# Dongwon-Lee/gkmQC

Measured on AMD Instinct MI355X. Metric: gkm kernel pairs/sec (N=10k, 300 bp, L=11,k=7,d=3), higher is better.
Workload: dtype u32

## Files before the change

gkmqc_amd/csrc/bitslice_cpu_probe.cpp:

```cpp
#include <stdint.h>
#include <stdlib.h>
#include <algorithm>
#include <vector>

#include "gkm_bitslice.h"
#include "gkm_pack.h"

using namespace gkmbs;

template <int W, int L, int D>
static void run_pair(const uint8_t *A, int lenA, const uint8_t *B, int lenB, const uint8_t *wd,
                     uint32_t *acc )
{
    constexpr int NB = planes_for(D);
    constexpr int CAP = segment_capacity(W, L);
    const int nA = lenA - L + 1, nB = lenB - L + 1, T = lenB;
    for (int k = 0; k <= D; k++) acc[k] = 0;
    (void)NB;
    std::vector<uint32_t> sb[2][3];
    for (int st = 0; st < 2; st++)
        for (int pl = 0; pl < 3; pl++) {
            sb[st][pl].resize((size_t)T + W);
            for (int x = 0; x < T + W; x++) sb[st][pl][(size_t)x] = sb_word(B, T, st, x, W, L, pl);
        }
// ... 15 lines not shown
        uint32_t lanepk[2 * W + 2];
        for (int x = 0; x < 2 * W + 2; x++) {
            uint32_t v = 0u;
            for (int k = 0; k < 16; k++) {
                const int pos = s0 + x * 16 + k;
                if (x * 16 + k < 32 * W && pos < lenA) v |= (uint32_t)A[pos] << (2 * k);
            }
            lanepk[x] = v;
        }
        auto rl = [&](int i0) { return pk_window(lanepk[i0 >> 4], lanepk[(i0 >> 4) + 1], i0); };
        auto cl = [&](int st, int q) { return pk_window(pkB[st][(size_t)(q >> 4)], pkB[st][(size_t)(q >> 4) + 1], q); };
        const int c0 = nA / 2 - s0;
        for (int st = 0; st < 2; st++)
            for (int delta = 0; delta < T; delta++) {
                uint32_t hit[W];
                window_hits<W, L, D>(Ahi, Alo, AV, &sb[st][0][(size_t)delta], &sb[st][1][(size_t)delta],
                                     (delta & 1) ? (const uint32_t *)nullptr : &sb[st][2][(size_t)delta], hit);
                for (int w = 0; w < W; w++) {
                    uint32_t h = hit[w];
                    while (h) {
                        const int bit = __builtin_ctz(h);
                        h &= h - 1u;
                        const HitValue hv = resolve_hit_packed<W>(bit, w, delta, st, (uint32_t)T, rcpT, nB, L, c0, rl, cl, wdist);
                        if (hv.m <= D) acc[hv.m] += hv.v;
                    }
                }
            }
    }
}

#define CASE(WW, LL, DD) \
    if (W == WW && L == LL && d == DD) { run_pair<WW, LL, DD>(A, lenA, B, lenB, wd, acc); ok = 1; }

extern "C" int bsprobe_profile(int W, int L, int d, const uint8_t *A, int lenA, const uint8_t *B, int lenB,
                               const uint8_t *wd, int32_t *P)
{
    uint32_t acc[16] = {0};
    int ok = 0;
    CASE(10, 11, 3) CASE(10, 10, 3) CASE(10, 12, 4) CASE(10, 8, 4) CASE(10, 9, 4) CASE(10, 12, 6) CASE(10, 11, 5) CASE(10, 12, 5)
    CASE(10, 4, 2) CASE(10, 2, 1) CASE(10, 3, 0) CASE(10, 5, 2) CASE(10, 6, 3) CASE(10, 7, 3)
    CASE(5, 11, 3) CASE(16, 11, 3) CASE(3, 12, 4) CASE(10, 12, 8) CASE(10, 12, 12) CASE(10, 11, 1)
    CASE(10, 9, 5) CASE(10, 10, 5) CASE(10, 10, 6) CASE(10, 11, 6) CASE(10, 11, 7) CASE(10, 12, 7)
    if (!ok) return 1;
    for (int m = 0; m <= d; m++) P[m] = (int32_t)acc[m];
    return 0;
}

template <int W, int L, int D, int GRP>
static void run_group_any(const uint32_t *Ahi, const uint32_t *Alo, const uint32_t *AV, const uint32_t *Bhi, const uint32_t *Blo,
                          uint32_t *hit_or, uint32_t *any)
{
    uint32_t hit[W];
    window_hits<W, L, D>(Ahi, Alo, AV, Bhi, Blo, (const uint32_t *)nullptr, hit);
    for (int g = 0; g < W / GRP; g++) {
        hit_or[g] = 0u;
        for (int k = 0; k < GRP; k++) hit_or[g] |= hit[g * GRP + k];
    }
    window_group_any<W, L, D, GRP>(Ahi, Alo, AV, Bhi, Blo, any);
}

#define GCASE(LL, DD) \
    if (L == LL && d == DD) { run_group_any<10, LL, DD, 5>(Ahi, Alo, AV, Bhi, Blo, hit_or, any); *top_plane = top_plane_serves(LL, DD) ? 1 : 0; return 0; }
#define GCASE_L(LL) GCASE(LL, 0) GCASE(LL, 1) GCASE(LL, 2) GCASE(LL, 3) GCASE(LL, 4)

extern "C" int bsprobe_group_any(int L, int d, const uint32_t *Ahi, const uint32_t *Alo, const uint32_t *AV, const uint32_t *Bhi,
                                 const uint32_t *Blo, uint32_t *hit_or, uint32_t *any, int *top_plane)
{
    GCASE_L(5) GCASE_L(6) GCASE_L(7) GCASE_L(8) GCASE_L(9) GCASE_L(10) GCASE_L(11) GCASE_L(12)
    GCASE(11, 5) GCASE(12, 5) GCASE(12, 6)
    return 1;
}

template <int W, int L, int D, int GRP>
static int run_group_any_grouped(const uint32_t *Ahi, const uint32_t *Alo, const uint32_t *AV, const uint32_t *Bhi,
                                 const uint32_t *Blo, uint32_t *any_grouped, uint32_t *top_or, uint32_t *avg)
{
    if constexpr (!top_plane_serves(L, D)) {
        return 2;
    } else {
        uint32_t ones[W];
        for (int w = 0; w < W; w++) ones[w] = 0xFFFFFFFFu;
        window_group_any<W, L, D, GRP>(Ahi, Alo, ones, Bhi, Blo, top_or);
        for (int g = 0; g < W / GRP; g++) {
            avg[g] = 0u;
            for (int k = 0; k < GRP; k++) avg[g] |= AV[g * GRP + k];
        }
        window_group_any_grouped<W, L, D, GRP>(Ahi, Alo, avg, Bhi, Blo, any_grouped);
        return 0;
    }
}

#define GGCASE(LL, DD) \
    if (L == LL && d == DD) return run_group_any_grouped<10, LL, DD, 5>(Ahi, Alo, AV, Bhi, Blo, any_grouped, top_or, avg);
#define GGCASE_L(LL) GGCASE(LL, 0) GGCASE(LL, 1) GGCASE(LL, 2) GGCASE(LL, 3) GGCASE(LL, 4)

extern "C" int bsprobe_group_any_grouped(int L, int d, const uint32_t *Ahi, const uint32_t *Alo, const uint32_t *AV,
                                         const uint32_t *Bhi, const uint32_t *Blo, uint32_t *any_grouped, uint32_t *top_or,
                                         uint32_t *avg)
{
    GGCASE_L(5) GGCASE_L(6) GGCASE_L(7) GGCASE_L(8) GGCASE_L(9) GGCASE_L(10) GGCASE_L(11) GGCASE_L(12)
    GGCASE(11, 5) GGCASE(12, 5) GGCASE(12, 6)
    return 1;
}

template <int W, int L, int D, int GRP>
static int run_group_any_crossings(const uint32_t *Ahi, const uint32_t *Alo, const uint32_t *AVg, const uint32_t *Bhi,
                                   const uint32_t *Blo, uint32_t *any_grouped, uint32_t *any_crossings, uint32_t *any_one_way)
{
    if constexpr (!top_plane_serves(L, D)) {
        return 2;
    } else {
        window_group_any_grouped<W, L, D, GRP>(Ahi, Alo, AVg, Bhi, Blo, any_grouped);
        window_group_any_crossings<W, L, D, GRP>(Ahi, Alo, AVg, Bhi, Blo, any_crossings);
        window_group_any_crossings<W, L, D, GRP, false>(Ahi, Alo, AVg, Bhi, Blo, any_one_way);
        return 0;
    }
}

#define XCASE(LL, DD) \
    if (L == LL && d == DD) return run_group_any_crossings<10, LL, DD, 5>(Ahi, Alo, AVg, Bhi, Blo, any_grouped, any_crossings, any_one_way);
#define XCASE_L(LL) XCASE(LL, 0) XCASE(LL, 1) XCASE(LL, 2) XCASE(LL, 3) XCASE(LL, 4)

extern "C" int bsprobe_group_any_crossings(int L, int d, const uint32_t *Ahi, const uint32_t *Alo, const uint32_t *AVg,
                                           const uint32_t *Bhi, const uint32_t *Blo, uint32_t *any_grouped,
                                           uint32_t *any_crossings, uint32_t *any_one_way)
{
    XCASE_L(5) XCASE_L(6) XCASE_L(7) XCASE_L(8) XCASE_L(9) XCASE_L(10) XCASE_L(11) XCASE_L(12)
    XCASE(11, 5) XCASE(12, 5) XCASE(12, 6)
    return 1;
}

template <int W, int L, int D, int GRP>
static int run_group_any_centres(const uint32_t *Ahi, const uint32_t *Alo, const uint32_t *AVg, const uint32_t *Bhi,
                                 const uint32_t *Blo, uint32_t *any_grouped, uint32_t *any_centres)
{
    if constexpr (!top_plane_serves(L, D)) {
        return 2;
    } else {
        window_group_any_grouped<W, L, D, GRP>(Ahi, Alo, AVg, Bhi, Blo, any_grouped);
        window_group_any_centres<W, L, D, GRP>(Ahi, Alo, AVg, Bhi, Blo, any_centres);
        return 0;
    }
}

#define CCASE(LL, DD) \
    if (L == LL && d == DD) return run_group_any_centres<10, LL, DD, 5>(Ahi, Alo, AVg, Bhi, Blo, any_grouped, any_centres);
#define CCASE_L(LL) CCASE(LL, 0) CCASE(LL, 1) CCASE(LL, 2) CCASE(LL, 3) CCASE(LL, 4)

extern "C" int bsprobe_group_any_centres(int L, int d, const uint32_t *Ahi, const uint32_t *Alo, const uint32_t *AVg,
                                         const uint32_t *Bhi, const uint32_t *Blo, uint32_t *any_grouped, uint32_t *any_centres)
{
    CCASE_L(5) CCASE_L(6) CCASE_L(7) CCASE_L(8) CCASE_L(9) CCASE_L(10) CCASE_L(11) CCASE_L(12)
    CCASE(11, 5) CCASE(12, 5) CCASE(12, 6)
    return 1;
}

extern "C" void bsprobe_row_planes(const uint8_t *codes, int len, int s0, int W, int L, uint32_t *out)
{
    for (int pl = 0; pl < 3; pl++)
        for (int w = 0; w < W; w++) out[pl * W + w] = row_plane_word(codes, len, s0, w, W, L, pl);
}
extern "C" void bsprobe_sb_words(const uint8_t *codes, int T, int strand, int W, int L, int nx, uint32_t *hi, uint32_t *lo)
{
    for (int x = 0; x < nx; x++) {
        hi[x] = sb_word(codes, T, strand, x, W, L, 0);
        lo[x] = sb_word(codes, T, strand, x, W, L, 1);
    }
}
extern "C" void bsprobe_piece_valid(int b0, int nb, int cnt, int W, uint32_t *out)
{
    for (int w = 0; w < W; w++) {
        out[w] = 0u;
        for (int b = 0; b < 32; b++) out[w] |= piece_bit((const uint8_t *)nullptr, 0, b0, nb, 0, cnt, b, w, W, 2) << b;
    }
}

template <int W, int L, int D>
static int run_packed(const uint8_t *codes, const int64_t *off, const int *rows, int nrows, int col,
                      const uint8_t *wd, int32_t *P_out, int *lanes_used, int max_rows = gkmpack::MAX_ROWS, int own_mult = 1,
                      int rider_w = 0, int shift_trip = 0, long long *visits_out = nullptr)
{
    using namespace gkmpack;
    std::vector<int> nwin((size_t)nrows);
    for (int i = 0; i < nrows; i++) nwin[(size_t)i] = (int)(off[rows[i] + 1] - off[rows[i]]) - L + 1;
    const Packing P = pack_rows(rows, nwin.data(), nrows, W, L, max_rows, 0, own_mult, rider_w);
    *lanes_used = (int)P.lanes_used;
    std::vector<std::vector<int>> owned((size_t)nrows);
    for (int i = 0; i < nrows; i++) owned[(size_t)i].assign((size_t)nwin[(size_t)i], 0);
    std::vector<int> row_tile((size_t)nrows, -1);
    std::vector<int> lane_bits((size_t)P.ntiles * LANES, 0), lane_np((size_t)P.ntiles * LANES, 0);
    for (const Piece &pc : P.pieces) {
        if (pc.b0 < 0 || pc.nb <= 0 || pc.b0 + pc.nb > 32) return -1;
        if (pc.cnt <= 0 || pc.cnt > pc.nb * W - (L - 1)) return -2;
        if (pc.rider ? pc.b0 < lane_bits[(size_t)pc.lane] : pc.b0 != lane_bits[(size_t)pc.lane]) return -3;
        lane_bits[(size_t)pc.lane] = pc.b0 + pc.nb;
        if (++lane_np[(size_t)pc.lane] > MAX_PIECES) return -4;
        const int t = pc.lane / LANES;
        const int i = P.tile_out[(size_t)t * MAX_ROWS + pc.slot];
        if (i < 0 || i >= nrows || rows[i] != pc.row || P.tile_row[(size_t)t * MAX_ROWS + pc.slot] != pc.row) return -5;
        if (row_tile[(size_t)i] >= 0 && row_tile[(size_t)i] != t) return -6;
        row_tile[(size_t)i] = t;
        for (int k = 0; k < pc.cnt; k++) {
            if (pc.p0 + k >= nwin[(size_t)i]) return -7;
            owned[(size_t)i][(size_t)(pc.p0 + k)]++;
        }
    }
    for (int i = 0; i < nrows; i++)
        for (int v : owned[(size_t)i])
            if (v != 1) return -8;
    for (int t = 0; t < P.ntiles; t++)
        if (P.tile_nrows[(size_t)t] > MAX_ROWS) return -9;

    constexpr int NB = planes_for(D);
    (void)NB;
    const uint8_t *B = codes + off[col];
    const int T = (int)(off[col + 1] - off[col]), nB = T - L + 1;
    std::vector<uint32_t> sb[2][2];
    for (int st = 0; st < 2; st++)
        for (int pl = 0; pl < 2; pl++) {
            sb[st][pl].resize((size_t)T + W);
            for (int x = 0; x < T + W; x++) sb[st][pl][(size_t)x] = sb_word(B, T, st, x, W, L, pl);
        }
    auto wdist = [&](int Dd) { return wd ? (uint32_t)wd[Dd] : 1u; };
    const int pkw = (T + 15) / 16 + 1;
    std::vector<uint32_t> pkB[2];
    for (int st = 0; st < 2; st++) {
        pkB[st].resize((size_t)pkw);
        for (int x = 0; x < pkw; x++) pkB[st][(size_t)x] = pk_word(B, T, st, x);
    }
    const uint32_t rcpT = mod_magic((uint32_t)T);
    std::vector<uint32_t> acc((size_t)nrows * (D + 1), 0u);
    size_t pi = 0;
    while (pi < P.pieces.size()) {
        size_t pj = pi;
        while (pj < P.pieces.size() && P.pieces[pj].lane == P.pieces[pi].lane) pj++;
        uint32_t Ahi[W], Alo[W], AV[W], start_mask = 0u;
        uint32_t lanepk[2 * W + 2];
        for (int w = 0; w < W; w++) Ahi[w] = Alo[w] = AV[w] = 0u;
        for (int x = 0; x < 2 * W + 2; x++) lanepk[x] = 0u;
        for (size_t k = pi; k < pj; k++) {
            const Piece &pc = P.pieces[k];
            start_mask |= 1u << pc.b0;
            const uint8_t *seq = codes + off[pc.row];
            const int len = (int)(off[pc.row + 1] - off[pc.row]);
            for (int w = 0; w < W; w++)
                for (int b = 0; b < 32; b++) {
                    Ahi[w] |= piece_bit(seq, len, pc.b0, pc.nb, pc.p0, pc.cnt, b, w, W, 0) << b;
                    Alo[w] |= piece_bit(seq, len, pc.b0, pc.nb, pc.p0, pc.cnt, b, w, W, 1) << b;
                    AV[w] |= piece_bit(seq, len, pc.b0, pc.nb, pc.p0, pc.cnt, b, w, W, 2) << b;
                    const int i = b * W + w;
                    lanepk[i >> 4] |= ((piece_bit(seq, len, pc.b0, pc.nb, pc.p0, pc.cnt, b, w, W, 0) << 1) |
                                       piece_bit(seq, len, pc.b0, pc.nb, pc.p0, pc.cnt, b, w, W, 1)) << (2 * (i & 15));
                }
        }
        auto resolve = [&](int bit, int w, int delta, int st) -> int {
                        const Piece &pc = P.pieces[pi + (size_t)piece_of_bitrow(start_mask, bit)];
                        const uint8_t *seq = codes + off[pc.row];
                        const int len = (int)(off[pc.row + 1] - off[pc.row]), nA = len - L + 1;
                        auto rl = [&](int i0) { return pk_window(lanepk[i0 >> 4], lanepk[(i0 >> 4) + 1], i0); };
                        auto cl = [&](int s2, int q) { return pk_window(pkB[s2][(size_t)(q >> 4)], pkB[s2][(size_t)(q >> 4) + 1], q); };
                        const int c0 = nA / 2 - pc.p0 + pc.b0 * W;
                        (void)seq;
                        const HitValue hv = resolve_hit_packed<W>(bit, w, delta, st, (uint32_t)T, rcpT, nB, L, c0, rl, cl, wdist);
                        const int i = P.tile_out[(size_t)(pc.lane / LANES) * MAX_ROWS + pc.slot];
                        if (hv.m <= D) acc[(size_t)i * (D + 1) + hv.m] += hv.v;
                        else if (hv.v != 0u) return -20;
                        return 0;
        };
        if constexpr (W == 2 * SHIFT_GROUP_WORDS) {
            if (shift_trip > 0) {
                struct Rec { uint32_t any0, any1, origin; };
                uint32_t AVg[2] = {0u, 0u};
                for (int w = 0; w < W; w++) AVg[w / SHIFT_GROUP_WORDS] |= AV[w];
                for (int st = 0; st < 2; st++) {
                    std::vector<Rec> stack;
                    auto trip = [&](size_t c) -> int {
                        std::vector<Rec> top(stack.end() - (long)c, stack.end());
                        stack.resize(stack.size() - c);
                        for (Rec r : top) {
                            const ShiftVisit v = shift_record_visit(r.any0, r.any1);
                            const int delta = rec_delta(r.origin);
                            if (rec_w(r.origin) != 0) return -21;
                            uint32_t hit[W];
                            window_hits<W, L, D>(Ahi, Alo, AV, &sb[st][0][(size_t)delta], &sb[st][1][(size_t)delta],
                                                 (const uint32_t *)nullptr, hit);
                            for (int k = 0; k < SHIFT_GROUP_WORDS; k++)
                                if ((hit[v.w0 + k] >> v.bit) & 1u)
                                    if (const int rc = resolve((int)v.bit, (int)v.w0 + k, delta, st)) return rc;
                            if (visits_out) visits_out[1]++;
                            if (shift_record_live(r.any0, r.any1)) {
                                stack.push_back(r);
                                if (visits_out) visits_out[2]++;
                            }
                        }
                        return 0;
                    };
                    for (int delta = 0; delta < T; delta++) {
                        uint32_t any[2];
                        if constexpr (top_plane_serves(L, D))
                            window_group_any_centres<W, L, D, SHIFT_GROUP_WORDS>(Ahi, Alo, AVg, &sb[st][0][(size_t)delta],
                                                                                 &sb[st][1][(size_t)delta], any);
                        else
                            window_group_any<W, L, D, SHIFT_GROUP_WORDS>(Ahi, Alo, AV, &sb[st][0][(size_t)delta],
                                                                         &sb[st][1][(size_t)delta], any);
                        if (shift_record_live(any[0], any[1])) {
                            stack.push_back(Rec{any[0], any[1], pack_meta(delta, 0, 0)});
// ... 198 lines not shown
```

gkmqc_amd/csrc/gkm_bitslice.h:

```cpp
#ifndef GKM_BITSLICE_H
#define GKM_BITSLICE_H

#include <stdint.h>

#if defined(__HIPCC__)
#define GKM_HD __host__ __device__ __forceinline__
#else
#define GKM_HD inline
#endif

namespace gkmbs {

constexpr int planes_for(int d) { return d <= 1 ? 1 : d <= 3 ? 2 : d <= 7 ? 3 : 4; }

constexpr int segment_capacity(int W, int L) { return 32 * W - (L - 1); }

template <int TT>
GKM_HD uint32_t lop3(uint32_t a, uint32_t b, uint32_t c)
{
#if defined(__HIP_DEVICE_COMPILE__)
    return __builtin_amdgcn_bitop3_b32(a, b, c, TT);
#else
    uint32_t r = 0u;
    for (int k = 0; k < 8; k++)
// ... 285 lines not shown
                const uint32_t zout = Z[w - 1], zin = Z[w + L - 1];
                const uint32_t old0 = cnt.b[0];
                cnt.b[0] = lop3<TT_XOR3>(old0, zin, zout);
                uint32_t t = lop3<TT_BXC_AND_AXC>(old0, zin, zout);
#pragma unroll
                for (int i = 1; i < P; i++) {
                    const uint32_t old = cnt.b[i];
                    cnt.b[i] = old ^ t;
                    if (i + 1 < P) t = lop3<TT_A_AND_BXC>(t, old, zout);
                }
            }
            const uint32_t top = cnt.b[P - 1];
            if (w % GRP == 0) any[w / GRP] = top & AV[w];
            else any[w / GRP] = lop3<TT_A_OR_BC>(any[w / GRP], top, AV[w]);
        }
    }
}

template <int W, int L, int D, int GRP>
GKM_HD void window_group_any_grouped(const uint32_t *Ahi, const uint32_t *Alo, const uint32_t *AVg, const uint32_t *Bhi,
                                     const uint32_t *Blo, uint32_t *any)
{
    static_assert(L >= 2 && L <= 12, "L out of range");
    static_assert(W % GRP == 0, "a shift is a whole number of groups");
    static_assert(top_plane_serves(L, D), "the grouped form exists for the top-plane (L, D) pairs only");
    constexpr int P = bitlen(L);
    constexpr int BETA = top_plane_bias(L, D);
    constexpr int NX = W + L - 1;
    uint32_t Z[NX];
#pragma unroll
    for (int w = 0; w < W; w++) Z[w] = lop3<TT_NOT_A_OR_BXC>(Ahi[w] ^ Bhi[w], Alo[w], Blo[w]);
#pragma unroll
    for (int x = W; x < NX; x++) Z[x] = Z[x - W] >> 1;

    Cnt<P, L + BETA> cnt;
    static_assert(Cnt<P, L + BETA>::P == P && !Cnt<P, L + BETA>::OV, "the biased count fills exactly its planes");
    cnt.ovf = 0u;
    plane_sum_columns_biased<0, P, L + BETA, L, BETA == 1>(Z, cnt);
    uint32_t top[W];
#pragma unroll
    for (int w = 0; w < W; w++) {
        if (w > 0) {
            const uint32_t zout = Z[w - 1], zin = Z[w + L - 1];
            const uint32_t old0 = cnt.b[0];
            cnt.b[0] = lop3<TT_XOR3>(old0, zin, zout);
            uint32_t t = lop3<TT_BXC_AND_AXC>(old0, zin, zout);
#pragma unroll
            for (int i = 1; i < P; i++) {
                const uint32_t old = cnt.b[i];
                cnt.b[i] = old ^ t;
                if (i + 1 < P) t = lop3<TT_A_AND_BXC>(t, old, zout);
            }
        }
        top[w] = cnt.b[P - 1];
        if (w % GRP == GRP - 1) {
            const int w0 = w - (GRP - 1);
            uint32_t a = top[w0];
#pragma unroll
            for (int g = 1; g + 1 < GRP; g += 2) a = lop3<TT_OR3>(a, top[w0 + g], top[w0 + g + 1]);
            if (GRP % 2 == 0) a |= top[w0 + GRP - 1];
            any[w0 / GRP] = a & AVg[w0 / GRP];
        }
    }
}

constexpr int TT_AXB_OR_C = 0xBE;
constexpr int TT_AB_AND_C = 0xA8;

template <int P>
GKM_HD uint32_t count_step_crossing(uint32_t *lo, uint32_t zin, uint32_t zout, bool last)
{
    const uint32_t old0 = lo[0];
    if (!last) lo[0] = lop3<TT_XOR3>(old0, zin, zout);
    uint32_t t = lop3<TT_BXC_AND_AXC>(old0, zin, zout);
#pragma unroll
    for (int i = 1; i < P - 1; i++) {
        const uint32_t old = lo[i];
        if (!last) lo[i] = old ^ t;
        t = lop3<TT_A_AND_BXC>(t, old, zout);
    }
    return t;
}
template <int N>
GKM_HD uint32_t or_terms_and(uint32_t a, const uint32_t *t, uint32_t v)
{
#pragma unroll
    for (int i = 0; i + 1 < N; i += 2) a = lop3<TT_OR3>(a, t[i], t[i + 1]);
    if constexpr (N % 2 == 1) return lop3<TT_AB_AND_C>(a, t[N - 1], v);
    else return a & v;
}

template <int W, int L, int D, int GRP, bool MIDDLE = true>
GKM_HD void window_group_any_crossings(const uint32_t *Ahi, const uint32_t *Alo, const uint32_t *AVg, const uint32_t *Bhi,
                                       const uint32_t *Blo, uint32_t *any)
{
    static_assert(L >= 2 && L <= 12, "L out of range");
    static_assert(W == 2 * GRP && GRP >= 3, "a shift is two groups");
    static_assert(top_plane_serves(L, D), "the crossings form exists for the top-plane (L, D) pairs only");
    constexpr int P = bitlen(L);
    static_assert(P >= 2, "a top plane and at least one below it");
    constexpr int BETA = top_plane_bias(L, D);
    constexpr int NX = W + L - 1;
    constexpr int C = MIDDLE ? GRP : 0;
    uint32_t Z[NX];
#pragma unroll
    for (int w = 0; w < W; w++) Z[w] = lop3<TT_NOT_A_OR_BXC>(Ahi[w] ^ Bhi[w], Alo[w], Blo[w]);
#pragma unroll
    for (int x = W; x < NX; x++) Z[x] = Z[x - W] >> 1;

    Cnt<P, L + BETA> cnt;
    static_assert(Cnt<P, L + BETA>::P == P && !Cnt<P, L + BETA>::OV, "the biased count fills exactly its planes");
    cnt.ovf = 0u;
    plane_sum_columns_biased<0, P, L + BETA, L, BETA == 1>(Z + C, cnt);
    const uint32_t top = cnt.b[P - 1];
    uint32_t up[P - 1];
#pragma unroll
    for (int i = 0; i < P - 1; i++) up[i] = cnt.b[i];

    if constexpr (MIDDLE) {
        uint32_t dn[P - 1];
#pragma unroll
        for (int i = 0; i < P - 1; i++) dn[i] = cnt.b[i];
        uint32_t tu[GRP - 1], td[GRP];
#pragma unroll
        for (int s = 0; s < GRP - 1; s++) {
            const int w = C + 1 + s;
            tu[s] = count_step_crossing<P>(up, Z[w + L - 1], Z[w - 1], s == GRP - 2);
        }
#pragma unroll
        for (int s = 0; s < GRP; s++) {
            const int w = C - 1 - s;
            td[s] = count_step_crossing<P>(dn, Z[w], Z[w + L], s == GRP - 1);
        }
        any[1] = or_terms_and<GRP - 1>(top, tu, AVg[1]);
        any[0] = or_terms_and<GRP - 2>(lop3<TT_AXB_OR_C>(top, td[0], td[1]), td + 2, AVg[0]);
    } else {
        uint32_t t[W - 1];
#pragma unroll
        for (int w = 1; w < W; w++) t[w - 1] = count_step_crossing<P>(up, Z[w + L - 1], Z[w - 1], w == W - 1);
        any[0] = or_terms_and<GRP - 1>(top, t, AVg[0]);
        uint32_t e = top;
#pragma unroll
        for (int i = 0; i + 1 < GRP; i += 2) e = lop3<TT_XOR3>(e, t[i], t[i + 1]);
        if constexpr (GRP % 2 == 0) any[1] = or_terms_and<GRP - 1>(e, t + GRP, AVg[1]);
        else any[1] = or_terms_and<GRP - 2>(lop3<TT_AXB_OR_C>(e, t[GRP - 1], t[GRP]), t + GRP + 1, AVg[1]);
    }
}

constexpr int TT_A_ANDN_B = 0x30;
constexpr int TT_UP_OR_LEVEL_C = 0xB2;
constexpr int TT_A_ANDN_B_C = 0x20;
constexpr int TT_AND3 = 0x80;

template <int W, int L, int D, int GRP>
GKM_HD void window_group_any_centres(const uint32_t *Ahi, const uint32_t *Alo, const uint32_t *AVg, const uint32_t *Bhi,
                                     const uint32_t *Blo, uint32_t *any)
{
    static_assert(L >= 2 && L <= 12, "L out of range");
    static_assert(W == 2 * GRP && GRP == 5, "a shift is two groups of five: every window within two steps of its group's centre");
    static_assert(top_plane_serves(L, D), "the centres form exists for the top-plane (L, D) pairs only");
    constexpr int P = bitlen(L);
    static_assert(P >= 3, "a top plane, plane 0 and at least one between them");
    constexpr int BETA = top_plane_bias(L, D);
    constexpr int NX = W + L - 1;
    uint32_t Z[NX];
#pragma unroll
    for (int w = 0; w < W; w++) Z[w] = lop3<TT_NOT_A_OR_BXC>(Ahi[w] ^ Bhi[w], Alo[w], Blo[w]);
#pragma unroll
    for (int x = W; x < NX; x++) Z[x] = Z[x - W] >> 1;

#pragma unroll
    for (int g = 0; g < W / GRP; g++) {
        constexpr int HALF = GRP / 2;
        const int C = g * GRP + HALF;
        Cnt<P, L + BETA> cnt;
        static_assert(Cnt<P, L + BETA>::P == P && !Cnt<P, L + BETA>::OV, "the biased count fills exactly its planes");
        cnt.ovf = 0u;
        plane_sum_columns_biased<0, P, L + BETA, L, BETA == 1>(Z + C, cnt);
        const uint32_t pu = lop3<TT_A_ANDN_B>(Z[C + L + 1], Z[C + 1], Z[C + 1]);
        const uint32_t m1u = lop3<TT_UP_OR_LEVEL_C>(Z[C + L], Z[C], pu);
        const uint32_t m2u = lop3<TT_A_ANDN_B_C>(Z[C + L], Z[C], pu);
        const uint32_t pd = lop3<TT_A_ANDN_B>(Z[C - 2], Z[C + L - 2], Z[C + L - 2]);
        const uint32_t m1d = lop3<TT_UP_OR_LEVEL_C>(Z[C - 1], Z[C + L - 1], pd);
        const uint32_t m2d = lop3<TT_A_ANDN_B_C>(Z[C - 1], Z[C + L - 1], pd);
        const uint32_t u = lop3<TT_AB_AND_C>(m1u, m1d, cnt.b[0]);
        uint32_t x = lop3<TT_OR3>(m2u, m2d, u);
#pragma unroll
        for (int i = 1; i + 1 <= P - 2; i += 2) x = lop3<TT_AND3>(cnt.b[i], cnt.b[i + 1], x);
        if constexpr ((P - 2) % 2 == 1) x &= cnt.b[P - 2];
        any[g] = lop3<TT_AB_AND_C>(cnt.b[P - 1], x, AVg[g]);
    }
}

GKM_HD uint32_t row_plane_word(const uint8_t *codes, int len, int s0, int w, int W, int L, int plane)
{
    uint32_t v = 0u;
    const int cap = 32 * W - (L - 1);
    for (int b = 0; b < 32; b++) {
        const int i = b * W + w, pos = s0 + i;
        uint32_t bit;
        if (plane == 2) bit = (pos <= len - L && i < cap) ? 1u : 0u;
        else bit = (pos < len) ? ((uint32_t)(codes[pos] >> (1 - plane)) & 1u) : 0u;
        v |= bit << b;
    }
    return v;
}

GKM_HD uint32_t piece_bit(const uint8_t *codes, int len, int b0, int nb, int p0, int cnt, int b, int w, int W,
                          int plane)
{
    if (b < b0 || b >= b0 + nb) return 0u;
    const int li = (b - b0) * W + w;
    if (plane == 2) return li < cnt ? 1u : 0u;
    const int pos = p0 + li;
    return pos < len ? ((uint32_t)(codes[pos] >> (1 - plane)) & 1u) : 0u;
}
GKM_HD int piece_of_bitrow(uint32_t start_mask, int b)
{
    return __builtin_popcount(start_mask & (0xFFFFFFFFu >> (31 - b))) - 1;
}

GKM_HD uint32_t sb_word(const uint8_t *codes, int T, int strand, int x, int W, int L, int plane)
{
    uint32_t v = 0u;
    int q = x % T;
    const int step = W % T;
    for (int b = 0; b < 32; b++) {
        uint32_t bit;
        if (plane == 2) bit = (q <= T - L) ? 1u : 0u;
        else {
            const uint32_t code = strand ? (3u - codes[T - 1 - q]) : codes[q];
            bit = (code >> (1 - plane)) & 1u;
        }
        v |= bit << b;
        q += step;
        if (q >= T) q -= T;
    }
    return v;
}

GKM_HD uint32_t mod_magic(uint32_t T) { return 0xFFFFFFFFu / T + 1u; }
GKM_HD uint32_t mod_small(uint32_t x, uint32_t T, uint32_t rcp)
{
#if defined(__HIP_DEVICE_COMPILE__)
    return x - __umulhi(x, rcp) * T;
#else
    return x - (uint32_t)(((uint64_t)x * rcp) >> 32) * T;
#endif
}

GKM_HD uint32_t dist_weight(const uint8_t *wd, int center, int p)
{
    const int dd = center - p;
    return wd[dd < 0 ? -dd : dd];
}

GKM_HD uint32_t lmer_entry(const uint8_t *codes, int len, int L, int strand, int p, uint32_t weight)
{
    uint32_t v = 0u;
    for (int i = 0; i < L; i++) {
        const uint32_t c = strand ? (3u - codes[len - 1 - (p + i)]) : codes[p + i];
        v = (v << 2) | c;
    }
    return v | (weight << 24);
}
GKM_HD int lmer_mismatch(uint32_t x, uint32_t y)
{
    uint32_t t = (x ^ y) & 0x00FFFFFFu;
    t = (t | (t >> 1)) & 0x00555555u;
    return __builtin_popcount(t);
}

struct HitValue {
    int m;
    uint32_t v;
};
template <int W, class RowLm, class ColLm>
GKM_HD HitValue resolve_hit(int b, int w, int delta, int strand, uint32_t T, uint32_t rcpT, int nB, RowLm rowlm,
                            ColLm collm)
{
    HitValue r;
    const int i0 = b * W + w;
    const uint32_t x = (uint32_t)(i0 + delta);
    int q;
    if (T >= (uint32_t)(32 * W)) {
        const uint32_t y = x - T;
        q = (int)(y < x ? y : x);
    } else {
        q = (int)mod_small(x, T, rcpT);
    }
    if (q >= nB) {
        r.m = 0;
        r.v = 0u;
        return r;
    }
    const uint32_t ea = rowlm(i0), eb = collm(strand, q);
    r.m = lmer_mismatch(ea, eb);
    r.v = (ea >> 24) * (eb >> 24);
    return r;
}

GKM_HD uint32_t pk_word(const uint8_t *codes, int len, int strand, int x)
{
    uint32_t v = 0u;
    for (int k = 0; k < 16; k++) {
        const int i = x * 16 + k;
        if (i >= len) break;
        const uint32_t c = strand ? (3u - codes[len - 1 - i]) : codes[i];
        v |= c << (2 * k);
    }
    return v;
}
GKM_HD uint32_t pk_word_cyclic(const uint8_t *codes, int len, int strand, int x)
{
    uint32_t v = 0u;
    int i = (x * 16) % len;
    for (int k = 0; k < 16; k++) {
        const uint32_t c = strand ? (3u - codes[len - 1 - i]) : codes[i];
        v |= c << (2 * k);
        if (++i == len) i = 0;
    }
    return v;
}
GKM_HD uint32_t pk_window(uint32_t lo, uint32_t hi, int pos)
{
#if defined(__HIP_DEVICE_COMPILE__)
    return __builtin_amdgcn_alignbit(hi, lo, (uint32_t)(2 * (pos & 15)));
#else
    return (uint32_t)((((uint64_t)hi << 32) | lo) >> (2 * (pos & 15)));
#endif
}
GKM_HD int pk_mismatch(uint32_t a, uint32_t b, int L)
{
    uint32_t t = (a ^ b) & ((1u << (2 * L)) - 1u);
    t = (t | (t >> 1)) & 0x55555555u;
    return __builtin_popcount(t);
}

template <int W, class RowWin, class ColWin, class Wdist>
GKM_HD HitValue resolve_hit_packed(int b, int w, int delta, int strand, uint32_t T, uint32_t rcpT, int nB, int L, int c0,
                                   RowWin roww, ColWin colw, Wdist wdist)
{
    HitValue r;
// ... 65 lines not shown
```

gkmqc_amd/csrc/gkm_gram_bitslice.hip:

```cpp
#include "gkm_gram_bitslice.h"

__device__ __forceinline__ uint32_t twice(uint32_t x)
{
    uint32_t r;
    asm("v_add_u32 %0, %1, %1" : "=v"(r) : "v"(x));
    return r;
}

#ifndef GKM_BS_GRP
#define GKM_BS_GRP 5
#endif
constexpr int BS_GRP = GKM_BS_GRP;
#ifndef GKM_BS_TRIP
#define GKM_BS_TRIP 64
#endif
constexpr int BS_TRIP = GKM_BS_TRIP;
static_assert(BS_TRIP == 64, "a trip resolves one record per lane");
constexpr int BS_CAP = BS_TRIP + 64;
#ifndef GKM_BS_WAVES
#define GKM_BS_WAVES 7
#endif
#ifndef GKM_BS_PACKED_WAVES
#define GKM_BS_PACKED_WAVES 6
#endif
#ifndef GKM_BS_CROSSINGS_MIDDLE
#define GKM_BS_CROSSINGS_MIDDLE 1
#endif
#ifndef GKM_BS_CENTRES
#define GKM_BS_CENTRES 1
#endif
#ifndef GKM_TRIP_PRIO
#define GKM_TRIP_PRIO 3
#endif

template <int W, int L, int D, int PK>
__global__ __launch_bounds__(64, D > 4 ? 1 : (PK >= 4 && PK <= 7) ? GKM_BS_WAVES : GKM_BS_PACKED_WAVES) void k_gram_bitslice(const BsArgs A)
{
    constexpr bool PACKED = PK == 1 || PK == 2;
    constexpr bool UNIF = PK >= 4 && PK <= 7;
    constexpr bool RIDERS = PK == 5 || PK == 7;
    constexpr bool SHIFTREC = PK == 6 || PK == 7;
    static_assert(PACKED || UNIF, "PK = 4 .. 7, 1 or 2");
    static_assert(!SHIFTREC || W == 2 * gkmbs::SHIFT_GROUP_WORDS, "a shift record holds the two groups of a shift");
    static_assert(L >= 5, "the L - 1 zero bytes either side of a weight table cover a group of five windows");
    using namespace gkmbs;
    extern __shared__ uint32_t s_dyn[];
    constexpr int NP = PACKED ? gkmpack::MAX_PIECES : 1;
    constexpr int NSLOT = (PK == 2 || RIDERS) ? gkmpack::MAX_ROWS : 64;
    constexpr int SSLOT = RIDERS ? gkmpack::RIDER_SLOTS : NSLOT;
    static_assert(gkmpack::RIDER_SLOTS <= gkmpack::MAX_ROWS, "the riders' row slots have profiles");
    constexpr int LIST_ARRAYS = SHIFTREC ? 3 : 2;
    constexpr int ACC_WORDS = (D + 1) * NSLOT, LIST_WORDS = LIST_ARRAYS * BS_CAP;
    constexpr int LPIECE_WORDS = PACKED ? 64 * NP : RIDERS ? 64 : 0;
    constexpr int STATIC_WORDS = ACC_WORDS + LIST_WORDS + LPIECE_WORDS;
    static_assert(!UNIF || STATIC_WORDS * 4 == bs_same_length_static_lds(PK, D), "gkm_gram_bitslice.h prices this LDS for the plan");
    __shared__ uint32_t s_mem[STATIC_WORDS];
    uint32_t *const accl = s_mem;
    uint32_t *const s_list = s_mem + ACC_WORDS;
    uint32_t *const lpiece = s_list + LIST_WORDS;
    static_assert((ACC_WORDS * 4) % 256 == 0, "the list's arrays stay 64-dword aligned (ds_write2st64_b32)");
    constexpr bool COL_BASE_FOLDS = (STATIC_WORDS * 4) % 1024 == 0;
    static_assert(W % BS_GRP == 0, "a shift is a whole number of record groups");
    static_assert(BS_CAP >= BS_TRIP + 64 && BS_CAP % 64 == 0, "hit list too small");
    static_assert(gkmpack::MAX_ROWS % 64 == 0, "row slots are finished 64 at a time");

    const int lane = threadIdx.x;
    int tile, j0;
    if (A.nent > 0) {
        int lo = 0, hi = A.nent;
        while (hi - lo > 1) {
            const int mid = (lo + hi) >> 1;
            if (A.ent_off[mid] <= (int64_t)blockIdx.x) lo = mid;
            else hi = mid;
        }
        tile = A.ent_tile[lo];
        j0 = A.ent_j0[lo] + (int)((int64_t)blockIdx.x - A.ent_off[lo]);
        if (j0 >= A.ent_j1[lo]) return;
    } else {
        int lo = 0, hi = A.ntiles;
        while (hi - lo > 1) {
            const int mid = (lo + hi) >> 1;
            if (A.tile_soff[mid] <= (int64_t)blockIdx.x) lo = mid;
            else hi = mid;
        }
        tile = lo;
        j0 = A.tile_cbeg[tile] + (int)((int64_t)blockIdx.x - A.tile_soff[tile]);
    }
    const int j1 = j0 + 1;
    const int nrows = A.tile_nrows[tile];
    constexpr int NE = NSLOT / 64;
    const bool two_copies = 2 * nrows <= NSLOT;

    uint32_t Ahi[W], Alo[W], AV[W];
#pragma unroll
    for (int w = 0; w < W; w++) {
        Ahi[w] = A.rowplanes[(((size_t)tile * 3 + 0) * W + w) * 64 + lane];
        Alo[w] = A.rowplanes[(((size_t)tile * 3 + 1) * W + w) * 64 + lane];
        AV[w] = A.rowplanes[(((size_t)tile * 3 + 2) * W + w) * 64 + lane];
    }
    constexpr bool GROUP_VALID = UNIF && gkmbs::top_plane_serves(L, D);
    uint32_t AVg[W / BS_GRP];
    if constexpr (GROUP_VALID) {
#pragma unroll
        for (int g = 0; g < W / BS_GRP; g++) {
            AVg[g] = AV[g * BS_GRP];
#pragma unroll
            for (int k = 1; k < BS_GRP; k++) AVg[g] |= AV[g * BS_GRP + k];
        }
    }

    uint32_t my_lmask = 0u;
    if (PACKED) {
        my_lmask = A.lane_mask[tile * 64 + lane];
#pragma unroll
        for (int k = 0; k < NP; k++) lpiece[lane * NP + k] = A.lane_piece[(size_t)(tile * 64 + lane) * NP + k];
    }
    const uint32_t lane_tag = ((uint32_t)lane << META_LANE_SHIFT) | (UNIF ? A.lane_piece[(size_t)(tile * 64 + lane) * 2] : 0u);
    if (RIDERS) lpiece[lane] = A.lane_piece[(size_t)(tile * 64 + lane) * 2 + 1];
    const uint32_t lane4 = (uint32_t)lane << 2;
    const int pkw = A.pkw;
    uint32_t *const s_col = s_dyn;
    uint8_t *const s_wtab = (uint8_t *)(s_dyn + 2 * pkw);
    const char *const rowpk_tile = (const char *)(A.rowpk + (size_t)tile * 64 * A.rpw);

    for (int j = j0; j < j1; j++) {
        const int T = A.len[j];
        const int nB = T - L + 1;
        const uint32_t rcpT = mod_magic((uint32_t)T);
        for (int x = lane; x < 2 * pkw; x += 64) s_col[x] = A.colpk[(size_t)j * 2 * pkw + x];
        uint32_t s_rowbase;
        for (int x = lane; x < A.ptw; x += 64) ((uint32_t *)s_wtab)[x] = A.postab[(size_t)j * A.ptw_stride + x];
        if (PACKED) {
            for (int x = lane; x < A.wdc_words; x += 64) ((uint32_t *)(s_wtab + A.ptw * 4))[x] = A.wdc[x];
            s_rowbase = (uint32_t)(STATIC_WORDS * 4) + (uint32_t)pkw * 8u + (uint32_t)A.ptw * 4u + (uint32_t)A.wdc_centre + 2048u;
        } else {
            s_rowbase = (uint32_t)(STATIC_WORDS * 4) + (uint32_t)pkw * 8u + POSTAB_PAD + (uint32_t)(L - 1);
        }
        uint32_t s_strand4 = 0u, s_wsign = 0u, s_wbase = 0u, s_wback = 0u, s_perm4 = 0x03020100u, s_perm1 = 0x0c0c0c04u;
#pragma unroll
        for (int m = 0; m <= D; m++)
            for (int rs = lane; rs < (two_copies ? NSLOT : nrows); rs += 64) accl[m * NSLOT + rs] = 0u;
        int s_n = 0;

        auto trip = [&](auto partial_tag, int c) {
            constexpr bool PARTIAL = decltype(partial_tag)::value;
            __builtin_amdgcn_s_setprio(GKM_TRIP_PRIO);
            const uint32_t top4 = (uint32_t)__builtin_amdgcn_readfirstlane((s_n - c) << 2);
            uint32_t at_off;
            asm("v_add_u32 %0, %1, %2" : "=v"(at_off) : "s"(top4), "v"(lane4));
            const char *const at = (const char *)s_list + at_off;
            uint32_t any = *(const uint32_t *)at;
            uint32_t any1 = SHIFTREC ? *(const uint32_t *)(at + BS_CAP * 4) : 0u;
            const uint32_t ms = *(const uint32_t *)(at + (LIST_ARRAYS - 1) * BS_CAP * 4);
            if (PARTIAL) any = (lane < c) ? any : 0u;
            if (PARTIAL && SHIFTREC) any1 = (lane < c) ? any1 : 0u;
            uint32_t bit, rw0, rest, live;
            if constexpr (SHIFTREC) {
                rest = any;
                any |= any1;
                const ShiftVisit sv = shift_record_visit(rest, any1);
                bit = sv.bit;
                rw0 = sv.w0;
                live = rest | any1;
            } else {
                bit = lowest_bit_or_ones(any);
                rest = any & (any - 1u);
                rw0 = ms & 15u;
                live = rest;
            }
            const uint32_t lane128 = ms & (63u << META_LANE_SHIFT);
            uint32_t lm = 0u;
            if (PACKED) lm = (uint32_t)__builtin_amdgcn_ds_bpermute((int)(lane128 >> 5), (int)my_lmask);
            uint32_t rtag = 0u;
            if (RIDERS) rtag = *(const uint32_t *)((const char *)lpiece + (lane128 >> 5));
            if (!PARTIAL || any) {
                const uint32_t i0 = __umul24(bit, (uint32_t)W) + rw0;
                uint32_t slot4, ia, nv = 5u;
                if (PACKED) {
                    const uint32_t below = lm & (0xFFFFFFFFu >> (31u - bit));
                    const uint32_t k = (uint32_t)__builtin_popcount(below) - 1u;
                    const uint32_t b0 = 31u - (uint32_t)__builtin_clz(below);
                    const uint32_t lp = *(const uint32_t *)((const char *)lpiece + ((lane128 >> 3) + (k << 2)));
                    slot4 = (lp << 2) & 0x1FCu;
                    const uint32_t c0b = (lp >> 7) & 0x1FFFu;
                    nv = (lp >> 20) - (i0 - __umul24(b0, (uint32_t)W));
                    ia = (i0 - c0b) + s_rowbase;
                } else if (RIDERS) {
                    const bool rides = bit >= (uint32_t)gkmpack::RIDER_B0;
                    const uint32_t res4 = (ms >> (META_SLOT_SHIFT - 2)) & 0x1FCu;
                    const uint32_t res_base = __umul24((ms >> META_PIECE_SHIFT) & 7u, (uint32_t)A.cap);
                    slot4 = rides ? (rtag & 0x1FCu) : res4;
                    ia = (rides ? (uint32_t)((int32_t)rtag >> RIDER_TAG_POS_SHIFT) : res_base) + i0 + s_rowbase;
                } else {
                    slot4 = (ms >> (META_SLOT_SHIFT - 2)) & 0xFCu;
                    ia = __umul24((ms >> META_PIECE_SHIFT) & 7u, (uint32_t)A.cap) + i0 + s_rowbase;
                }
                const uint32_t x = i0 + (ms >> 21);
                uint32_t q;
                if ((uint32_t)T >= (uint32_t)(32 * W)) q = min(x - (uint32_t)T, x);
                else q = mod_small(x, (uint32_t)T, rcpT);
                const uint32_t *rw = (const uint32_t *)(rowpk_tile + lop3<0xEA>(i0 >> 2, ~3u, lane128));
                typedef const uint32_t __attribute__((address_space(3))) *lds_words;
                const uint32_t cwo = lop3<0xEA>(q >> 1, ~7u, s_strand4);
                const lds_words cw = COL_BASE_FOLDS ? (lds_words)(uintptr_t)cwo : (lds_words)(uintptr_t)((uint32_t)(STATIC_WORDS * 4) + cwo);
                const uint32_t ib = (q ^ s_wsign) + s_wbase;
                const uint32_t il = ib - s_wback;
                const lds_words pa = (lds_words)(uintptr_t)(ia & ~3u);
                const lds_words pb = (lds_words)(uintptr_t)(il & ~3u);
                const uint32_t a0 = pa[0], a1 = pa[1], b0 = pb[0], b1 = pb[1];
                const uint32_t sha = (ia & 3u) << 3, shb = (il & 3u) << 3;
                uint32_t wa4 = __builtin_amdgcn_alignbit(a1, a0, sha), wa1 = a1 >> sha;
                if (PACKED) {
                    wa4 &= 0xFFFFFFFFu >> (32u - 8u * min(nv, 4u));
                    wa1 = nv >= 5u ? wa1 : 0u;
                }
                const uint32_t lo = __builtin_amdgcn_alignbit(b1, b0, shb), hi = b1 >> shb;
                const uint32_t wb4 = __builtin_amdgcn_perm(hi, lo, s_perm4), wb1 = __builtin_amdgcn_perm(hi, lo, s_perm1);
                const uint32_t ea = __builtin_amdgcn_alignbit(rw[1], rw[0], twice(i0));
                const uint32_t eb = __builtin_amdgcn_alignbit(cw[2], cw[0], twice(q));
                uint32_t t = ea ^ eb;
                t = (t | (t >> 1)) & 0x55555555u;
                static_assert(5 + L - 1 <= 16, "the five windows of a group lie inside one 16-base window");
#pragma unroll
                for (int k = 0; k < 5; k++) {
                    const uint32_t m = (uint32_t)__builtin_popcount(__builtin_amdgcn_ubfe(t, 2u * k, 2u * L));
                    const uint32_t wa = k < 4 ? ((wa4 >> (8 * k)) & 0xFFu) : (wa1 & 0xFFu);
                    const uint32_t wb = k < 4 ? ((wb4 >> (8 * k)) & 0xFFu) : (wb1 & 0xFFu);
                    if (m <= (uint32_t)D)
                        atomicAdd((uint32_t *)((char *)accl + (m * (uint32_t)(NSLOT * 4) + slot4)), wa * wb);
                }
            }
            s_n -= c;
            const unsigned long long more = __ballot(live != 0u);
            if (more) {
                const uint32_t rank = __builtin_amdgcn_mbcnt_hi((uint32_t)(more >> 32),
                                                                __builtin_amdgcn_mbcnt_lo((uint32_t)more, 0u));
                if (live != 0u) {
                    char *const to = (char *)s_list + ((rank + (uint32_t)s_n) << 2);
                    *(uint32_t *)to = rest;
                    if (SHIFTREC) *(uint32_t *)(to + BS_CAP * 4) = any1;
                    *(uint32_t *)(to + (LIST_ARRAYS - 1) * BS_CAP * 4) = ms;
                }
                s_n += (int)__popcll(more);
            }
            __builtin_amdgcn_s_setprio(0);
        };

        auto trips = [&](bool final) {
            while (s_n >= BS_TRIP) trip(std::false_type(), BS_TRIP);
            if (final)
                while (s_n > 0) {
                    if (s_n >= BS_TRIP) trip(std::false_type(), BS_TRIP);
                    else trip(std::true_type(), s_n);
                }
        };

        for (int strand = 0; strand < 2; strand++) {
            s_strand4 = (uint32_t)strand * 4u + (COL_BASE_FOLDS ? (uint32_t)(STATIC_WORDS * 4) : 0u);
            s_wsign = strand ? ~0u : 0u;
            s_wback = strand ? 4u : 0u;
            s_perm4 = strand ? 0x01020304u : 0x03020100u;
            s_perm1 = strand ? 0x0c0c0c00u : 0x0c0c0c04u;
            s_wbase = (uint32_t)(STATIC_WORDS * 4) + (uint32_t)pkw * 8u + POSTAB_PAD + (uint32_t)(L - 1) + (strand ? (uint32_t)nB : 0u);
            const sgpr_words sbh = (sgpr_words)(A.sb + ((size_t)(j * 2 + strand) * 2) * A.xw);
            const sgpr_words sbl = sbh + A.xw;
            for (int d0 = 0; d0 < T; d0 += BS_DU) {
                uint32_t bh[BS_DU + W - 1], bl[BS_DU + W - 1];
#pragma unroll
                for (int i = 0; i < BS_DU + W - 1; i++) {
                    bh[i] = sbh[d0 + i];
                    bl[i] = sbl[d0 + i];
                }
#pragma unroll
                for (int u = 0; u < BS_DU; u++) {
                    if (d0 + u < T) {
                        uint32_t grp_any[W / BS_GRP];
                        if constexpr (GROUP_VALID && SHIFTREC && GKM_BS_CENTRES != 0)
                            window_group_any_centres<W, L, D, BS_GRP>(Ahi, Alo, AVg, bh + u, bl + u, grp_any);
                        else if constexpr (GROUP_VALID && SHIFTREC)
                            window_group_any_crossings<W, L, D, BS_GRP, GKM_BS_CROSSINGS_MIDDLE != 0>(Ahi, Alo, AVg, bh + u, bl + u, grp_any);
                        else if constexpr (GROUP_VALID)
                            window_group_any_grouped<W, L, D, BS_GRP>(Ahi, Alo, AVg, bh + u, bl + u, grp_any);
                        else
                            window_group_any<W, L, D, BS_GRP>(Ahi, Alo, AV, bh + u, bl + u, grp_any);
                        uint32_t s_delta = pack_meta(d0 + u, 0, 0);
                        asm("" : "+s"(s_delta));
                        const uint32_t vbase = lane_tag | s_delta;
                        if constexpr (SHIFTREC) {
                            static_assert(W / BS_GRP == 2 && BS_GRP == gkmbs::SHIFT_GROUP_WORDS, "a shift record is two groups of five");
                            const uint32_t any0 = grp_any[0], any1 = grp_any[1];
                            const bool hit = shift_record_live(any0, any1);
                            const unsigned long long mask = __ballot(hit);
                            const int rank = (int)__builtin_amdgcn_mbcnt_hi((uint32_t)(mask >> 32),
                                                                            __builtin_amdgcn_mbcnt_lo((uint32_t)mask, 0u));
                            if (hit) {
                                char *const at = (char *)s_list + (((uint32_t)rank + (uint32_t)s_n) << 2);
                                *(uint32_t *)at = any0;
                                *(uint32_t *)(at + BS_CAP * 4) = any1;
                                *(uint32_t *)(at + 2 * BS_CAP * 4) = vbase;
                            }
                            s_n += (int)__popcll(mask);
                            if (s_n >= BS_TRIP) trips(false);
                        } else {
#pragma unroll
                        for (int w0 = 0; w0 < W; w0 += BS_GRP) {
                            const uint32_t any = grp_any[w0 / BS_GRP];
                            const unsigned long long mask = __ballot(any != 0u);
                            const int rank = (int)__builtin_amdgcn_mbcnt_hi((uint32_t)(mask >> 32),
                                                                            __builtin_amdgcn_mbcnt_lo((uint32_t)mask, 0u));
                            if (any != 0u) {
                                char *const at = (char *)s_list + (((uint32_t)rank + (uint32_t)s_n) << 2);
                                *(uint32_t *)at = any;
                                *(uint32_t *)(at + BS_CAP * 4) = vbase | (uint32_t)w0;
                            }
                            s_n += (int)__popcll(mask);
                            if (s_n >= BS_TRIP) trips(false);
                        }
                        }
                    }
                }
            }
            trips(true);
        }

#pragma unroll
        for (int k = 0; k < NE; k++) {
            const int rs = k * 64 + lane;
            const int row = rs < nrows ? A.tile_row[tile * gkmpack::MAX_ROWS + rs] : -1;
            if (row < 0 || (j > row && !A.out.write_all)) continue;
            uint32_t prof[D + 1];
#pragma unroll
            for (int m = 0; m <= D; m++) prof[m] = accl[m * NSLOT + rs] + (two_copies ? accl[m * NSLOT + rs + NSLOT / 2] : 0u);
            double g = 0.0;
#pragma unroll
            for (int m = 0; m <= D; m++) g += A.c[m] * (double)(int32_t)prof[m];
            const int64_t r = A.out.local_rows ? A.tile_out[tile * gkmpack::MAX_ROWS + rs] : row;
            if (A.out.diag && j == row) A.out.diag[row] = g;
            if (A.S) A.S[(A.tile_soff[tile] + (j - A.tile_cbeg[tile])) * SSLOT + rs] = g;
            if (A.out.P) {
#pragma unroll
                for (int m = 0; m <= D; m++)
                    A.out.P[(r * A.out.ldp + j) * (D + 1) + m] = (int32_t)prof[m];
            }
        }
    }
}

template <int W, int PACKED>
static bs_kernel_t pick_bitslice(int L, int d)
{
#define GKM_BS(LL, DD) \
    if (L == LL && d == DD) { \
        if constexpr ((PACKED != 5 && PACKED != 7) || LL - 1 <= gkmpack::RIDER_NB * W - gkmpack::RIDER_W) return k_gram_bitslice<W, LL, DD, PACKED>; \
        else return nullptr;  \
    }
#define GKM_BS_L(LL) GKM_BS(LL, 0) GKM_BS(LL, 1) GKM_BS(LL, 2) GKM_BS(LL, 3) GKM_BS(LL, 4)
    GKM_BS_L(5) GKM_BS_L(6) GKM_BS_L(7) GKM_BS_L(8) GKM_BS_L(9) GKM_BS_L(10) GKM_BS_L(11) GKM_BS_L(12)
    GKM_BS(11, 5) GKM_BS(12, 5) GKM_BS(12, 6)
#undef GKM_BS_L
#undef GKM_BS
    return nullptr;
}

bs_kernel_t gkm_pick_bitslice(int pk, int L, int d)
{
    switch (pk) {
    case 1: return pick_bitslice<10, 1>(L, d);
    case 2: return pick_bitslice<10, 2>(L, d);
    case 4: return pick_bitslice<10, 4>(L, d);
    case 5: return pick_bitslice<10, 5>(L, d);
    case 6: return pick_bitslice<10, 6>(L, d);
    case 7: return pick_bitslice<10, 7>(L, d);
    }
    return nullptr;
}
```

Baseline: 1.070 billion.

## Share overlapping column-sum inputs between the two centre groups and fold top planes

The centre-based group test now precompresses the Z words that both groups' window counts overlap into shared sum/carry terms through 3:2 compressors. Each group's popcount then starts from its own five words plus these shared partials, so the overlap is not recounted. When the top two planes come from a two-input column, the final threshold test folds them with a majority op instead of building the top plane. The kernel default switches to this shared form, and a CPU probe entry compares the shared and private forms against the grouped reference.

```diff
diff --git a/gkmqc_amd/csrc/bitslice_cpu_probe.cpp b/gkmqc_amd/csrc/bitslice_cpu_probe.cpp
--- a/gkmqc_amd/csrc/bitslice_cpu_probe.cpp
+++ b/gkmqc_amd/csrc/bitslice_cpu_probe.cpp
@@ -191,6 +191,33 @@
 {
     CCASE_L(5) CCASE_L(6) CCASE_L(7) CCASE_L(8) CCASE_L(9) CCASE_L(10) CCASE_L(11) CCASE_L(12)
     CCASE(11, 5) CCASE(12, 5) CCASE(12, 6)
+    return 1;
+}
+
+template <int W, int L, int D, int GRP>
+static int run_group_any_centres_forms(const uint32_t *Ahi, const uint32_t *Alo, const uint32_t *AVg, const uint32_t *Bhi,
+                                       const uint32_t *Blo, uint32_t *any_grouped, uint32_t *any_shared, uint32_t *any_private)
+{
+    if constexpr (!top_plane_serves(L, D)) {
+        return 2;
+    } else {
+        window_group_any_grouped<W, L, D, GRP>(Ahi, Alo, AVg, Bhi, Blo, any_grouped);
+        window_group_any_centres<W, L, D, GRP>(Ahi, Alo, AVg, Bhi, Blo, any_shared);
+        window_group_any_centres<W, L, D, GRP, false>(Ahi, Alo, AVg, Bhi, Blo, any_private);
+        return 0;
+    }
+}
+
+#define FCASE(LL, DD) \
+    if (L == LL && d == DD) return run_group_any_centres_forms<10, LL, DD, 5>(Ahi, Alo, AVg, Bhi, Blo, any_grouped, any_shared, any_private);
+#define FCASE_L(LL) FCASE(LL, 0) FCASE(LL, 1) FCASE(LL, 2) FCASE(LL, 3) FCASE(LL, 4)
+
+extern "C" int bsprobe_group_any_centres_forms(int L, int d, const uint32_t *Ahi, const uint32_t *Alo, const uint32_t *AVg,
+                                               const uint32_t *Bhi, const uint32_t *Blo, uint32_t *any_grouped,
+                                               uint32_t *any_shared, uint32_t *any_private)
+{
+    FCASE_L(5) FCASE_L(6) FCASE_L(7) FCASE_L(8) FCASE_L(9) FCASE_L(10) FCASE_L(11) FCASE_L(12)
+    FCASE(11, 5) FCASE(12, 5) FCASE(12, 6)
     return 1;
 }
 
diff --git a/gkmqc_amd/csrc/gkm_bitslice.h b/gkmqc_amd/csrc/gkm_bitslice.h
--- a/gkmqc_amd/csrc/gkm_bitslice.h
+++ b/gkmqc_amd/csrc/gkm_bitslice.h
@@ -461,7 +461,26 @@
 constexpr int TT_A_ANDN_B_C = 0x20;
 constexpr int TT_AND3 = 0x80;
 
-template <int W, int L, int D, int GRP>
+constexpr bool top_pair_folds(int I, int P, int N)
+{
+    return I > P - 2 ? false : I == P - 2 ? N == 2 : top_pair_folds(I + 1, P, N / 2);
+}
+template <int I, int P, int N, bool FOLD>
+GKM_HD void centre_planes(const uint32_t *x, uint32_t *b, uint32_t *pq)
+{
+    if constexpr (FOLD && I == P - 2) {
+        static_assert(N == 2, "the fold is for a column of exactly two planes");
+        pq[0] = x[0];
+        pq[1] = x[1];
+    } else if constexpr (I < P) {
+        static_assert(N >= 1, "a plane of the count has at least one input");
+        uint32_t carry[ColumnSum<N>::NC > 0 ? ColumnSum<N>::NC : 1];
+        b[I] = ColumnSum<N>::run(x, carry);
+        centre_planes<I + 1, P, ColumnSum<N>::NC, FOLD>(carry, b, pq);
+    }
+}
+
+template <int W, int L, int D, int GRP, bool SHARED = true>
 GKM_HD void window_group_any_centres(const uint32_t *Ahi, const uint32_t *Alo, const uint32_t *AVg, const uint32_t *Bhi,
                                      const uint32_t *Blo, uint32_t *any)
 {
@@ -472,32 +491,82 @@
     static_assert(P >= 3, "a top plane, plane 0 and at least one between them");
     constexpr int BETA = top_plane_bias(L, D);
     constexpr int NX = W + L - 1;
+    constexpr int HALF = GRP / 2;
     uint32_t Z[NX];
 #pragma unroll
     for (int w = 0; w < W; w++) Z[w] = lop3<TT_NOT_A_OR_BXC>(Ahi[w] ^ Bhi[w], Alo[w], Blo[w]);
 #pragma unroll
     for (int x = W; x < NX; x++) Z[x] = Z[x - W] >> 1;
 
+    constexpr bool SH = SHARED && L >= GRP;
+    constexpr int OV0 = GRP + HALF;
+    constexpr int NOV = SH ? L - GRP : 0;
+    constexpr int NF = NOV / 3, REST = NOV - 3 * NF;
+    constexpr bool BIAS_SH = SH && BETA == 1 && REST > 0;
+    constexpr int NS = NF + (BIAS_SH ? 1 : REST), NY = NF + (BIAS_SH ? 1 : 0);
+    constexpr int N0 = GRP + NS;
+    constexpr bool CIN0 = BETA == 1 && !BIAS_SH;
+    using CS0 = ColumnSumBiased<N0, CIN0>;
+    constexpr int N1 = CS0::NC + NY;
+    constexpr bool FOLD = SH && top_pair_folds(1, P, N1);
+    uint32_t ss[NS > 0 ? NS : 1], sy[NY > 0 ? NY : 1];
+    if constexpr (SH) {
+#pragma unroll
+        for (int i = 0; i < NF; i++) {
+            const uint32_t a = Z[OV0 + 3 * i], b = Z[OV0 + 3 * i + 1], c = Z[OV0 + 3 * i + 2];
+            ss[i] = lop3<TT_XOR3>(a, b, c);
+            sy[i] = lop3<TT_MAJ>(a, b, c);
+        }
+        if constexpr (BIAS_SH && REST == 2) {
+            const uint32_t a = Z[OV0 + 3 * NF], b = Z[OV0 + 3 * NF + 1];
+            ss[NF] = lop3<TT_XNOR_AB>(a, b, b);
+            sy[NF] = a | b;
+        } else if constexpr (BIAS_SH) {
+            ss[NF] = ~Z[OV0 + 3 * NF];
+            sy[NF] = Z[OV0 + 3 * NF];
+        } else {
+#pragma unroll
+            for (int i = 0; i < REST; i++) ss[NF + i] = Z[OV0 + 3 * NF + i];
+        }
+    }
+
 #pragma unroll
     for (int g = 0; g < W / GRP; g++) {
-        constexpr int HALF = GRP / 2;
         const int C = g * GRP + HALF;
-        Cnt<P, L + BETA> cnt;
-        static_assert(Cnt<P, L + BETA>::P == P && !Cnt<P, L + BETA>::OV, "the biased count fills exactly its planes");
-        cnt.ovf = 0u;
-        plane_sum_columns_biased<0, P, L + BETA, L, BETA == 1>(Z + C, cnt);
+        uint32_t b[P], pq[2] = {0u, 0u};
+        if constexpr (SH) {
+            const int X0 = g == 0 ? HALF : HALF + L;
+            uint32_t c0[N0], c1[N1];
+#pragma unroll
+            for (int i = 0; i < GRP; i++) c0[i] = Z[X0 + i];
+#pragma unroll
+            for (int i = 0; i < NS; i++) c0[GRP + i] = ss[i];
+            b[0] = CS0::run(c0, c1);
+#pragma unroll
+            for (int i = 0; i < NY; i++) c1[CS0::NC + i] = sy[i];
+            centre_planes<1, P, N1, FOLD>(c1, b, pq);
+        } else {
+            Cnt<P, L + BETA> cnt;
+            static_assert(Cnt<P, L + BETA>::P == P && !Cnt<P, L + BETA>::OV, "the biased count fills exactly its planes");
+            cnt.ovf = 0u;
+            plane_sum_columns_biased<0, P, L + BETA, L, BETA == 1>(Z + C, cnt);
+#pragma unroll
+            for (int i = 0; i < P; i++) b[i] = cnt.b[i];
+        }
         const uint32_t pu = lop3<TT_A_ANDN_B>(Z[C + L + 1], Z[C + 1], Z[C + 1]);
         const uint32_t m1u = lop3<TT_UP_OR_LEVEL_C>(Z[C + L], Z[C], pu);
         const uint32_t m2u = lop3<TT_A_ANDN_B_C>(Z[C + L], Z[C], pu);
         const uint32_t pd = lop3<TT_A_ANDN_B>(Z[C - 2], Z[C + L - 2], Z[C + L - 2]);
         const uint32_t m1d = lop3<TT_UP_OR_LEVEL_C>(Z[C - 1], Z[C + L - 1], pd);
         const uint32_t m2d = lop3<TT_A_ANDN_B_C>(Z[C - 1], Z[C + L - 1], pd);
-        const uint32_t u = lop3<TT_AB_AND_C>(m1u, m1d, cnt.b[0]);
+        const uint32_t u = lop3<TT_AB_AND_C>(m1u, m1d, b[0]);
         uint32_t x = lop3<TT_OR3>(m2u, m2d, u);
-#pragma unroll
-        for (int i = 1; i + 1 <= P - 2; i += 2) x = lop3<TT_AND3>(cnt.b[i], cnt.b[i + 1], x);
-        if constexpr ((P - 2) % 2 == 1) x &= cnt.b[P - 2];
-        any[g] = lop3<TT_AB_AND_C>(cnt.b[P - 1], x, AVg[g]);
+        constexpr int TOPMID = FOLD ? P - 3 : P - 2;
+#pragma unroll
+        for (int i = 1; i + 1 <= TOPMID; i += 2) x = lop3<TT_AND3>(b[i], b[i + 1], x);
+        if constexpr (TOPMID >= 1 && TOPMID % 2 == 1) x &= b[TOPMID];
+        if constexpr (FOLD) any[g] = lop3<TT_MAJ>(pq[0], pq[1], x) & AVg[g];
+        else any[g] = lop3<TT_AB_AND_C>(b[P - 1], x, AVg[g]);
     }
 }
 
diff --git a/gkmqc_amd/csrc/gkm_gram_bitslice.hip b/gkmqc_amd/csrc/gkm_gram_bitslice.hip
--- a/gkmqc_amd/csrc/gkm_gram_bitslice.hip
+++ b/gkmqc_amd/csrc/gkm_gram_bitslice.hip
@@ -27,7 +27,7 @@
 #define GKM_BS_CROSSINGS_MIDDLE 1
 #endif
 #ifndef GKM_BS_CENTRES
-#define GKM_BS_CENTRES 1
+#define GKM_BS_CENTRES 2
 #endif
 #ifndef GKM_TRIP_PRIO
 #define GKM_TRIP_PRIO 3
@@ -276,7 +276,7 @@
                     if (d0 + u < T) {
                         uint32_t grp_any[W / BS_GRP];
                         if constexpr (GROUP_VALID && SHIFTREC && GKM_BS_CENTRES != 0)
-                            window_group_any_centres<W, L, D, BS_GRP>(Ahi, Alo, AVg, bh + u, bl + u, grp_any);
+                            window_group_any_centres<W, L, D, BS_GRP, GKM_BS_CENTRES == 2>(Ahi, Alo, AVg, bh + u, bl + u, grp_any);
                         else if constexpr (GROUP_VALID && SHIFTREC)
                             window_group_any_crossings<W, L, D, BS_GRP, GKM_BS_CROSSINGS_MIDDLE != 0>(Ahi, Alo, AVg, bh + u, bl + u, grp_any);
                         else if constexpr (GROUP_VALID)
```

Measured after the change: 1.132 billion, median of 6. 1.06x the previous value.
